# chechaohp/gan-ode

Hardware: AMD Instinct MI355X
Metric: generated videos/sec (16-frame clips) (higher is better)
Workload: dtype f32

## Files before the change

gan-ode_amd/_lib.py:

```python
from __future__ import annotations

import ctypes as C
import os

_HERE = os.path.dirname(os.path.abspath(__file__))
LIB_PATH = os.path.join(_HERE, "lib", "libgode.so")

i32, i64, f32, ptr = C.c_int32, C.c_int64, C.c_float, C.c_void_p
cint, u32, u64 = C.c_int, C.c_uint32, C.c_uint64

ACT_NONE, ACT_RELU, ACT_LRELU, ACT_TANH_OUT = 0, 1, 2, 3
ACT_TANH, ACT_SIGMOID = 4, 5
ACT_LRELU01 = 6
EPI_RAW, EPI_TANH = 0, 1
FPROP, DGRAD = 0, 1
PACK_BORDER = 0x100
OP_IGEMM, OP_WGRAD, OP_BN_FINALIZE, OP_BN_BWD, OP_ODE_FWD, OP_ODE_BWD, OP_BCE, OP_ADAM, OP_PACK = range(1, 10)
OP_ODERNN_FWD, OP_ODERNN_BWD, OP_BN_APPLY, OP_COL2IM = 10, 11, 12, 13
OP_SDE_FWD, OP_SDE_BWD = 14, 15
OP_CDE_FWD, OP_CDE_BWD = 16, 17
OP_WGAN = 18
OP_GRU_FWD, OP_GRU_BWD = 19, 20
OP_DNOISE = 21
OP_CATEG, OP_CE = 22, 23
OP_CHSTATS, OP_CBN_EMBED, OP_CBN_EMBED_BWD, OP_CBN_APPLY, OP_CBN_BWD, OP_GRES_OUT, OP_GRES_OUT_BWD, OP_SN_FWD, OP_SN_BWD = range(24, 33)
OP_FC_ACT, OP_FC_ACT_BWD, OP_BCE_PROB = 33, 34, 35
OP_BCE_T = 36
OP_RESIZE_U8, OP_CLIP_GATHER = 37, 38
RESIZE_MAX_TAPS = 32
REC_ADAM_NOISE = -1
ODE_NPARAM = 2672
ODERNN_NPARAM = 2176
SDE_NPARAM = 3216
CDE_NPARAM = 7536
CDE_MAX_N = 4096
GRU_NPARAM = 1632
# ... 315 lines not shown
    "gode_bn_bwd_work_size": ([i64, i32], i64),
    "gode_ode_bwd_work_size": ([i32], i64),
    "gode_odernn_bwd_work_size": ([i32], i64),
    "gode_odernn_sync_size": ([i32], i64),
    "gode_sde_bwd_work_size": ([i32], i64),
    "gode_cde_sync_size": ([i32], i64),
    "gode_cde_state_size": ([i32, i32], i64),
    "gode_cde_bwd_work_size": ([i32], i64),
    "gode_gru_bwd_work_size": ([i32], i64),
    "gode_ode_fwd_multi": ([ptr, i32, ptr], cint),
    "gode_ode_bwd_multi": ([ptr, i32, ptr], cint),
    "gode_odernn_fwd_multi": ([ptr, i32, ptr], cint),
    "gode_odernn_bwd_multi": ([ptr, i32, ptr], cint),
    "gode_odernn_fwd_route": ([ptr, i32, ptr], cint),
    "gode_odernn_bwd_route": ([ptr, i32, ptr], cint),
    "gode_gru_fwd_multi": ([ptr, i32, ptr], cint),
    "gode_gru_bwd_multi": ([ptr, i32, ptr], cint),
    "gode_chstats_rows": ([i64], cint),
    "gode_cbn_bwd_work_size": ([i32, i32, i32, i32], i64),
    "gode_gres_out_bwd_work_size": ([i32, i32, i32, i32, i32, i32], i64),
    "gode_fc_act_bwd_work_size": ([i64, i32], i64),
    "gode_dropout_mask": ([ptr, i64, u64, u32, f32, ptr], cint),
    "gode_scale": ([ptr, ptr, i64, f32, cint, ptr], cint),
    "gode_adam_multi": ([ptr, i32, i64, f32, f32, f32, f32, f32, f32, i32, ptr], cint),
    "gode_adam_multi_dev": ([ptr, i32, i64, f32, f32, f32, f32, f32, ptr, ptr], cint),
    "gode_adam_noise_multi": ([ptr, i32, i64, f32, f32, f32, f32, f32, f32, i32, u64, u32, u32, f32, ptr], cint),
    "gode_adam_noise_multi_dev": ([ptr, i32, i64, f32, f32, f32, f32, f32, ptr, u64, u32, f32, ptr], cint),
    "gode_param_noise": ([ptr, i64, u64, u32, u32, i64, f32, i32, ptr], cint),
    "gode_dnoise_normals": ([ptr, i64, u64, u32, u32, u32, i64, i32, ptr], cint),
    "gode_ode_step_chunks": ([ptr, i64], i64),
    "gode_ode_step": ([ptr, i32, i64, i32, f32, f32, f32, f32, f32, ptr, ptr], cint),
    "gode_axpy_multi": ([ptr, i32, i64, f32, ptr, ptr, f32, ptr, ptr, ptr], cint),
    "gode_run": ([ptr, ptr, i32, ptr], cint),
    "gode_version": (None, cint),
    "gode_sizeof": ([cint], cint),
}

EXPORTS = [st.FN for st in _OPS] + list(_PROTOS)

_lib = None


def lib():
    global _lib
    if _lib is not None:
        return _lib
    if not os.path.exists(LIB_PATH):
        raise RuntimeError(f"{LIB_PATH} is missing: build it with `python __graft_entry__.py` "
                           "(hipcc --offload-arch=gfx950); there is no CPU or PyTorch fallback")
    L = C.CDLL(LIB_PATH)
    for name in EXPORTS:
        if not hasattr(L, name):
            raise RuntimeError(f"libgode.so does not export {name}")
        fn = getattr(L, name)
        fn.argtypes, fn.restype = _PROTOS.get(name, ([ptr, ptr], cint))
    for kind, st in _STRUCTS.items():
        if L.gode_sizeof(kind) != C.sizeof(st):
            raise RuntimeError(f"ABI mismatch for op kind {kind}: C {L.gode_sizeof(kind)} != ctypes {C.sizeof(st)}")
    _lib = L
    return L


def check(rc, what="gode call"):
    if rc != 0:
        raise RuntimeError(f"{what} failed with code {rc}" + (" (hipError)" if rc > 0 else " (argument/shape error)"))


TRACE = None


def _traced(op, stream, launch):
    import torch
    e0, e1 = torch.cuda.Event(enable_timing=True), torch.cuda.Event(enable_timing=True)
    e0.record()
    launch()
    e1.record()
    TRACE.append((op, e0, e1))


def call(tag, launch):
    if TRACE is not None:
        return _traced(tag, None, launch)
    launch()


class Program:

    def __init__(self, ops):
        self.ops = list(ops)
        n = len(self.ops)
        self.kinds = (i32 * n)(*[op.KIND for op in self.ops])
        self.ptrs = (ptr * n)(*[C.addressof(op) for op in self.ops])
        self.n = n

    def run(self, stream):
        if TRACE is not None:
            for op in self.ops:
                run_one(op, stream)
            return
        check(lib().gode_run(self.kinds, self.ptrs, self.n, stream), "gode_run")


def run_one(op, stream):
    if op.KIND == OP_PACK:
        launch = lambda: check(lib().gode_pack_weights(C.byref(op.g), op.dir, op.w, op.wpack, op.co_perm, op.co_canon,
                                                       stream), "gode_pack_weights")
        return _traced(op, stream, launch) if TRACE is not None else launch()
    if TRACE is not None:
        return _traced(op, stream, lambda: _run_one(op, stream))
    _run_one(op, stream)


def _run_one(op, stream):
    check(getattr(lib(), op.FN)(C.byref(op), stream), op.FN)
```

gan-ode_amd/csrc/api.hip:

```cpp
#include "common.h"

extern "C" int gode_version(void) { return GODE_VERSION; }

extern "C" int gode_sizeof(int kind) {
  switch (kind) {
    case 0: return (int)sizeof(gode_conv_geom);
    case -1: return (int)sizeof(gode_adam_noise_tensor);
    case GODE_OP_PACK: return (int)sizeof(gode_pack_op);
#define GODE_SIZEOF_ROW_(name, value, op_t, fn) case GODE_OP_##name: return (int)sizeof(op_t);
    GODE_OPS(GODE_SIZEOF_ROW_)
#undef GODE_SIZEOF_ROW_
  }
  return GODE_E_KIND;
}

extern "C" int gode_pack_batch_(const gode_pack_op* const* ops, int n, void* stream);

extern "C" int gode_run(const int32_t* kinds, const void* const* ops, int32_t n, void* stream) {
  if (n < 0 || (n > 0 && (!kinds || !ops))) return GODE_E_ARG;
  for (int i = 0; i < n; ++i) {
    int rc;
    switch (kinds[i]) {
#define GODE_RUN_ROW_(name, value, op_t, fn) case GODE_OP_##name: rc = fn((const op_t*)ops[i], stream); break;
      GODE_OPS(GODE_RUN_ROW_)
#undef GODE_RUN_ROW_
      case GODE_OP_PACK: {
        int j = i;
        while (j + 1 < n && kinds[j + 1] == GODE_OP_PACK) ++j;
        rc = gode_pack_batch_((const gode_pack_op* const*)(ops + i), j - i + 1, stream);
        if (rc == 0) i = j;
        break;
      }
      default: return GODE_E_KIND;
    }
    if (rc != 0) return rc > 0 ? rc : rc * 1000 - i;
  }
  return 0;
}
```

gan-ode_amd/engine.py:

```python
from __future__ import annotations

import ctypes as C
import os
from dataclasses import dataclass
from typing import List, Optional, Sequence

import numpy as np
import torch

from . import _lib as L

BORDER_TAKE_DEAD_TAPS = 0.06
BORDER_TAKE_TILES_PER_SLOT = 2.0


def border_value(g) -> int:
    lib = L.lib()
    if lib.gode_igemm_dead_taps(C.byref(L.IgemmOp(g=g, dir=L.DGRAD, tile=0))) < BORDER_TAKE_DEAD_TAPS:
        return 1
    info = (C.c_int32 * 4)()
    L.check(lib.gode_igemm_launch_info(C.byref(L.IgemmOp(g=g, dir=L.DGRAD, tile=0, border=2)), info))
    return 2 if info[0] and info[2] >= BORDER_TAKE_TILES_PER_SLOT * info[3] else 1


def make_geom(N, Ci, Co, xi, yo, k, s, p) -> L.ConvGeom:
    return L.ConvGeom(N, Ci, Co, xi[0], xi[1], xi[2], yo[0], yo[1], yo[2], k[0], k[1], k[2], s[0], s[1], s[2],
                      p[0], p[1], p[2])


def conv_out(i, k, s, p):
    return (i + 2 * p - k) // s + 1


def dptr(t: Optional[torch.Tensor]):
    return None if t is None else t.data_ptr()


def stream_ptr():
    return torch.cuda.current_stream().cuda_stream


@dataclass
class LayerSpec:
    geom: L.ConvGeom
    fwd_dir: int
    act: int
    has_bn: bool
    epilogue: int = L.EPI_RAW
    co_perm: Optional[torch.Tensor] = None
    noise: bool = False

    def out_dims(self):
        g = self.geom
        if self.fwd_dir == L.FPROP:
            return (g.N, g.Do, g.Ho, g.Wo, g.Co)
        return (g.N, g.Di, g.Hi, g.Wi, g.Ci)

    def in_dims(self):
        g = self.geom
        if self.fwd_dir == L.FPROP:
            return (g.N, g.Di, g.Hi, g.Wi, g.Ci)
        return (g.N, g.Do, g.Ho, g.Wo, g.Co)


@dataclass
class LayerParams:
    weight: torch.Tensor
    gamma: Optional[torch.Tensor] = None
    beta: Optional[torch.Tensor] = None
    running_mean: Optional[torch.Tensor] = None
    running_var: Optional[torch.Tensor] = None
    num_batches_tracked: Optional[torch.Tensor] = None
# ... 84 lines not shown
        self._param_ptrs = None

    def _shared_pack(self, l, direction, n):
        key = ("buf", l, direction)
        buf = self.pack_cache.get(key)
        if buf is None or buf.numel() != n or buf.device != torch.device(self.device):
            buf = self.pack_cache[key] = torch.empty(n, dtype=torch.float32, device=self.device)
            self.pack_cache.pop(("ver", l, direction), None)
        return buf

    def _attach_work(self, igemm_ops):
        lib = L.lib()
        need = max([lib.gode_igemm_work_size(C.byref(op)) for op in igemm_ops] + [0])
        if need > 0:
            if self._ig_work is None or self._ig_work.numel() < need:
                self._ig_work = torch.empty(need, dtype=torch.float32, device=self.device)
                for prog_ops in getattr(self, "_all_igemm", []):
                    for op in prog_ops:
                        op.work = self._ig_work.data_ptr()
            for op in igemm_ops:
                op.work = self._ig_work.data_ptr()
        self.__dict__.setdefault("_all_igemm", []).append(list(igemm_ops))

    def _run_stale_packs(self, packs, st):
        stale = []
        for l, d, op in packs:
            w = self.params[l].weight
            ver = (w._version, getattr(w, "_gode_ver", 0), w.data_ptr())
            if self.pack_cache.get(("ver", l, d)) != ver:
                self.pack_cache[("ver", l, d)] = ver
                stale.append(op)
        if stale:
            L.Program(stale).run(st)

    @staticmethod
    def _ncols(s: LayerSpec):
        g = s.geom
        if s.fwd_dir == L.FPROP:
            return g.Co
        fullk = (g.Do == 1 and g.Ho == 1 and g.Wo == 1 and g.pd == 0 and g.ph == 0 and g.pw == 0 and
                 g.Di == g.kd and g.Hi == g.kh and g.Wi == g.kw and g.kd * g.kh * g.kw > 1)
        return g.kd * g.kh * g.kw * g.Ci if fullk else g.Ci

    def _materialize(self, l):
        if l + 1 >= len(self.specs):
            return False
        if self.specs[l + 1].noise:
            return True
        prod, cons = self.specs[l], self.specs[l + 1]
        C_out = prod.out_dims()[4]
        g = cons.geom
        taps = g.kd * g.kh * g.kw
        macs = g.N * g.Do * g.Ho * g.Wo * g.Co * g.Ci * taps
        heavy = C_out % 32 == 0 and macs >= (1 << 30) and (prod.has_bn or prod.act != L.ACT_NONE)
        if self._G2 and prod.has_bn:
            if self.split and not heavy and l + 1 == self.nl - 1 and cons.epilogue == L.EPI_TANH and not cons.has_bn:
                self._last_parts = True
                return False
            return True
        return heavy

    def _head_as_gemm(self, l):
        s = self.specs[l]
        g = s.geom
        taps = g.kh * g.kw
        pixels = g.N * g.Ho * g.Wo
# ... 223 lines not shown
                    continue
                ops.append(L.BnApplyOp(y=dptr(self.y[l]), out=dptr(self.a[l]), scale=dptr(self.scale[l]),
                                       shift=dptr(self.shift[l]), M=M, C=d[4], act=s.act, M0=M0))
        patch["packs"] = packs
        self._attach_work([op for op in ops if isinstance(op, L.IgemmOp)])
        return L.Program(ops), patch

    def _noise_op(self, noise, l, scale, shift, M0):
        d = self.specs[l].out_dims()
        op = L.DnoiseOp(x=dptr(self.y[l]), out=dptr(self.a[l]), scale=scale, shift=shift, M=d[0] * d[1] * d[2] * d[3],
                        C=d[4], act=self.specs[l].act, M0=M0, layer=l + 1)
        noise.append((op, d[1] * d[2] * d[3] * d[4], 0, None))
        return op

    @staticmethod
    def _patch_noise(patch, noise, inputs):
        seed = int(noise["seed"]) & 0xFFFFFFFFFFFFFFFF
        seed = seed - (1 << 64) if seed >= 1 << 63 else seed
        dev = noise.get("call_dev")
        base = 0 if dev else int(noise["call"])
        for op, per, add, k in patch["noise"]:
            op.seed, op.stream, op.sigma = seed, int(noise["stream"]), float(noise["sigma"])
            c = (base + add) & 0xFFFFFFFF
            op.call_dev, op.call = dev, c - (1 << 32) if c >= 1 << 31 else c
            op.e_off = int(noise.get("sample_offset", 0)) * per
            if k is not None:
                x, xs = inputs[k]
                op.x = x.data_ptr()
                for i in range(5):
                    op.xs[i] = int(xs[i])

    def forward(self, training: bool, x: Optional[torch.Tensor] = None, x_strides=None, pre_ops_program=None,
                x2: Optional[torch.Tensor] = None, x2_strides=None, noise=None):
        self._refresh()
        if training not in self._fwd:
            self._fwd[training] = self._build_fwd(training)
        prog, patch = self._fwd[training]
        if self.noisy:
            if noise is None:
                raise RuntimeError("this plan applies instance noise: forward() needs its noise arguments")
            self._patch_noise(patch, noise, [(x, x_strides), (x2, x2_strides)])
        out = torch.empty(self.out_dims, dtype=torch.float32, device=self.device)
        patch["last"].out = out.data_ptr()
        if "last2" in patch:
            patch["last2"][0].out = out.data_ptr() + patch["last2"][1]
        if self.x_in is None and self.x0n is None:
            first = patch["first"]
            first.src = x.data_ptr()
            for i in range(5):
                first.gs[i] = int(x_strides[i])
        if self.x_in is None:
            self._x_user, self._x_strides = x.detach(), tuple(int(v) for v in x_strides)
            if self.groups == 2:
                if self.x0n is None:
                    second = patch["first2"]
                    second.src = x2.data_ptr()
                    for i in range(5):
                        second.gs[i] = int(x2_strides[i])
                self._x2_user, self._x2_strides = x2.detach(), tuple(int(v) for v in x2_strides)
        st = stream_ptr()
        self._run_stale_packs(patch["packs"], st)
        if pre_ops_program is not None:
            pre_ops_program.run(st)
        prog.run(st)
        self.out = out.detach()
        self.generation += 1
        self._fwd_training = training
        return out

    def n_grad_floats(self):
        n = 0
        for p in self.params:
            n += p.weight.numel()
            if p.gamma is not None:
                n += p.gamma.numel() + p.beta.numel()
        return n

    def _build_bwd(self, need_input_grad: bool, need_param_grad: bool = True, training: bool = True):
        lib = L.lib()
        f32 = dict(dtype=torch.float32, device=self.device)
        if self.g is None:
            self.g = [torch.empty(s.out_dims(), **f32) for s in self.specs]
            self.g_in = None
        ops, patch = [], {"dw": [], "dgamma": [], "dbeta": []}
        bpacks = []
        wg_work = 0
        bn_work = 0
        last = self.specs[-1]
        readers = patch["gout_readers"] = []
        if last.epilogue == L.EPI_TANH:
            M = self._count(self.nl - 1)
            op = L.BnBwdOp(g=dptr(self.g[-1]), y=None, M=M, C=last.out_dims()[4], act=L.ACT_TANH_OUT)
            patch["tanh"] = op
            readers.append((op, "gin"))
            ops.append(op)
        for l in range(self.nl - 1, -1, -1):
            s, p = self.specs[l], self.params[l]
# ... 229 lines not shown
```

gan-ode_amd/modules.py:

```python
from __future__ import annotations

import ctypes as C
import math
from typing import Optional

import numpy as np
import torch
import torch.nn as nn

from . import _lib as L
from .engine import ConvStack, LayerParams, LayerSpec, conv_out, dptr, make_geom, stream_ptr

Z_COLS = 96
Z_CATEG0 = 66
MAX_CATEG = Z_COLS - Z_CATEG0
ODE_METHODS = L.ODE_METHODS


def ode_method_code(name):
    return L.ode_method_code(name)


def _require_gpu(t: torch.Tensor, what: str):
    if not t.is_cuda:
        raise RuntimeError(f"{what}: this implementation runs only on an MI355X through libgode.so; move the module "
                           "to the GPU with .cuda() (there is no CPU or PyTorch fallback)")


class _Pool:

    MAX_PLANS = 6

    def __init__(self):
        self.plans = {}
        self.pack_cache = {}

    def get(self, key, factory):
        lst = self.plans.setdefault(key, [])
        for p in lst:
            if not p.busy:
                return p
        if len(lst) >= self.MAX_PLANS:
            p = lst.pop(0)
            p.busy = False
            lst.append(p)
            return p
        p = factory()
        lst.append(p)
        return p
# ... 165 lines not shown
    multi, multi_always = ("ode", L.OdeFwdOp, L.OdeBwdOp), False

    def __init__(self, gen: "VideoGenerator", n_traj: int, T: int, select: bool, zbuf=None, x=None):
        dev = gen.main[0].weight.device
        self.gen, self.n, self.T, self.select, self.device = gen, n_traj, T, select, dev
        self.rows = n_traj if select else n_traj * T
        f32 = dict(dtype=torch.float32, device=dev)
        self.ncat = int(getattr(gen, "dim_z_category", 0)) if x is None else 0
        self.labels = None
        self.x, self.content, self.sel, self.cls = x, None, None, None
        self._ring = []
        if x is None:
            xs = self._x_shape(n_traj, T)
            sx, sc, ss, sk = _input_slices(int(np.prod(xs)), n_traj)
            nin = sk.stop if self.ncat else sk.start
            self._in = torch.zeros(nin, **f32)
            self.x, self.content = self._in[sx].view(xs), self._in[sc].view(n_traj, 50)
            self.sel = self._in[ss].view(torch.int32) if select else None
            self.cls = self._in[sk].view(torch.int32) if self.ncat else None
            self._ring = [dict(buf=torch.zeros(nin).pin_memory(), ev=None) for _ in range(4)]
        self._ring_i = 0
        self.stack = None
        if x is not None:
            self._zbuf, self._zcols = torch.empty(n_traj * T, self.zcols, **f32), self.zcols
        elif zbuf is not None:
            self._zbuf, self._zcols = zbuf, Z_COLS
        else:
            self.stack = ConvStack(gen._decoder_specs(self.rows), gen._decoder_params(), dev, owns_input=True,
                                   pack_cache=gen._pool.pack_cache, two_lane_backward=True)
            self._zbuf, self._zcols = self.stack.x_in, Z_COLS
        self._alloc()
        self._ode_ptrs = None
        self.busy = False

    @staticmethod
    def _x_shape(n_traj, T):
        return (n_traj, 16)

    def _alloc(self):
        f32 = dict(dtype=torch.float32, device=self.device)
        self.traj = torch.empty(self.n, self.T, 16, **f32)
        tt = torch.linspace(0, 1, self.T).float()
        self.dt = (tt[1:] - tt[:-1]).to(self.device) if self.T > 1 else torch.zeros(1, **f32)
        self.ode_work = torch.empty(L.lib().gode_ode_bwd_work_size(self.n), **f32)

    def _params(self):
        g = self.gen
        lin = g.linear
        if isinstance(lin, nn.Identity):
            pre = (None, None, None, None)
        else:
            pre = (lin[0].weight, lin[0].bias, lin[2].weight, lin[2].bias)
        return pre + tuple(_ode_fn_tensors(g.ode_fn))

    @classmethod
    def multi_ok(cls, gen, adjoint):
        if cls.multi is None:
            return False
        return cls.multi_always or (gen.ode_method == "dopri5" and not (adjoint and gen.adjoint_substeps != 0))

    def check_solve(self):
        """Host-side look at a finished solve (the CDE plan's: it raises when the kernel stopped early)."""

    def latent_rows(self):
        if self.rows_in_traj:
            return self.traj.view(self.n * self.T, 16)
# ... 52 lines not shown
                                          rows_per=1 if self.select else self.T, C=self.ncat, zcols=zcols, col0=Z_CATEG0)
            self.fwd_prog = L.Program([self.fwd_op] + ([self.categ_op] if self.ncat else []))
        self.fwd_op.substeps = self.bwd_op.substeps = self.gen.ode_substeps
        if self.gen.ode_method == "dopri5":
            self.bwd_op.substeps = self.gen.adjoint_substeps

    def stage_inputs(self, x_host, content_host, sel_host, cls_host=None):
        self._programs()
        if self.ncat:
            if cls_host is None:
                raise RuntimeError("a categorical generator plan needs the classes of its trajectories")
            if getattr(self.gen, "_feed", None) is not None and self.gen._feed.recording:
                raise NotImplementedError("categorical latents are not captured in a graph (GanTrainer(graph=True))")
            if not self.select:
                self.labels = torch.empty(self.n, dtype=torch.int64, device=self.device)
            self.categ_op.labels_out = dptr(self.labels) if not self.select else None
        feed = getattr(self.gen, "_feed", None)
        if feed is not None and feed.recording:
            nfl = self._in.numel()
            pin, dev = feed.noise_region(self.gen, self.select, self.n, self.T, nfl)
            _pack_inputs(pin, x_host, content_host, sel_host, cls_host)
            self._in.copy_(dev)
        else:
            slot = self._ring[self._ring_i]
            self._ring_i = (self._ring_i + 1) % len(self._ring)
            if slot["ev"] is not None:
                slot["ev"].synchronize()
            _pack_inputs(slot["buf"], x_host, content_host, sel_host, cls_host)
            self._in.copy_(slot["buf"], non_blocking=True)
            if slot["ev"] is None:
                slot["ev"] = torch.cuda.Event()
            slot["ev"].record()

    def forward(self, x_host, content_host, sel_host, training, keep, cls_host=None):
        if x_host is None:
            torch.cuda.current_stream().wait_event(self._latent_ev)
            out = self.stack.forward(training)
        else:
            self.stage_inputs(x_host, content_host, sel_host, cls_host)
            out = self.stack.forward(training, pre_ops_program=self.fwd_prog)
        self.busy = keep
        return out

    def _decoder_pass_done(self):
        cb = getattr(self.gen, "_on_decoder_grads", None)
        if cb is not None:
            self.gen._decoder_passes_left -= 1
            if self.gen._decoder_passes_left == 0:
                cb()

    def backward(self, gout, arena=None):
        if arena is not None:
            into = _grads_into(arena, self.gen._decoder_params())
            _, _, gz = self.stack.backward(gout, need_input_grad=True, into=into)
            self._decoder_pass_done()
            self.latent_backward(gz.data_ptr(), arena, gz)
            self.busy = False
            return None, None
        flat, views, gz = self.stack.backward(gout, need_input_grad=True)
        motion = self.latent_backward(gz.data_ptr(), None, gz)
        self.busy = False
        return views, motion

    def latent_backward(self, gz_ptr, arena, keep):
        op = self.bwd_op
        op.gz = gz_ptr
        ps = self._params()
        absent = _PRENET_NPARAM if ps[0] is None else 0
        cut = absent if self.grads_from_first_present else 0
        if arena is not None:
            tgt = [arena.target(q) for q in ps if q is not None]
            base, acc = tgt[0]
            op.grads = base.data_ptr() - 4 * (absent - cut)
            op.accumulate = 1 if acc else 0
            batch = getattr(self.gen, "_adjoint_batch", None)
# ... 69 lines not shown
        return (None,) * (n_other + ctx.n_params)
    views, motion = plan.backward(gout, None)
    grads = _flat_grads(views)
    assert len(grads) == ctx.n_dec and len(motion) == ctx.n_params - ctx.n_dec
    return (None,) * n_other + (*grads, *motion)


class _GenJointFn(torch.autograd.Function):

    @staticmethod
    def forward(ctx, plan, host, training, keep, n_dec, *params):
        out = plan.forward(host, training, keep)
        ctx.plan, ctx.n_dec, ctx.n_params = plan, n_dec, len(params)
        ctx.lease = _Lease(plan)
        ctx.out_shape = tuple(out.shape)
        return out.narrow(0, 0, plan.rows_v), out.narrow(0, plan.rows_v, plan.rows_i)

    @staticmethod
    def backward(ctx, gv, gi):
        plan = ctx.plan
        ctx.lease.check(type(plan.gen).__name__ + " (joint pass)")
        g = torch.empty(ctx.out_shape, dtype=torch.float32, device=plan.device)
        for part, gg in ((g.narrow(0, 0, plan.rows_v), gv), (g.narrow(0, plan.rows_v, plan.rows_i), gi)):
            if gg is None:
                part.zero_()
            else:
                part.copy_(gg)
        return _gen_backward(ctx, plan, g, 5)


class _GenFn(torch.autograd.Function):

    @staticmethod
    def forward(ctx, plan, x_host, content_host, sel_host, cls_host, training, keep, n_dec, *params):
        out = plan.forward(x_host, content_host, sel_host, training, keep, cls_host)
        ctx.plan, ctx.n_dec, ctx.n_params = plan, n_dec, len(params)
        ctx.lease = _Lease(plan)
        return out

    @staticmethod
    def backward(ctx, gout):
        plan = ctx.plan
        ctx.lease.check(type(plan.gen).__name__)
        return _gen_backward(ctx, plan, gout, 8)


class _LatentFn(torch.autograd.Function):

    @staticmethod
    def forward(ctx, gen, x_host, n, T, *params):
        lp = gen._plan_cls(gen, n, T, False, x=x_host.to(gen.main[0].weight.device))
        lp._programs()
        lp.fwd_prog.run(stream_ptr())
        lp.check_solve()
        ctx.lp = lp
        return lp.latent_rows()

    @staticmethod
    def backward(ctx, gout):
        lp = ctx.lp
        g = gout.contiguous()
        lp.bwd_op.zcols = 16
        return (None, None, None, None, *lp.latent_backward(g.data_ptr(), None, g))


class VideoGenerator(nn.Module):

    mnist = False
    _plan_cls = None
    _categorical_ok = True
    _one_layer_ok = True
    ode_method = "rk4"
    ode_rtol, ode_atol, adjoint_substeps = 1e-7, 1e-9, 0

    def __init__(self, n_channels, dim_z_content, dim_z_category, dim_z_motion, video_length, ode_fn=ODEFunc,
                 dim_hidden=None, linear=True, ngf=64):
        super().__init__()
        if not self._categorical_ok and dim_z_category != 0:
            raise NotImplementedError(f"categorical latents (dim_z_category={dim_z_category}) are implemented for the "
                                      f"Neural-ODE generators only, not for {type(self).__name__}")
        if not (0 <= int(dim_z_category) <= MAX_CATEG) or int(dim_z_category) != dim_z_category:
            raise NotImplementedError(f"dim_z_category={dim_z_category}: the categorical one-hot lives in the {MAX_CATEG} pad "
                                      f"columns of the {Z_COLS}-column latent row (0 <= dim_z_category <= {MAX_CATEG})")
        if dim_z_motion != 16 or dim_z_content != 50:
            raise NotImplementedError("libgode's fused ODE kernels are specialised for dim_z_motion=16, "
                                      "dim_z_content=50 (mnist_moco_ode.py:78, ucf_moco_ode.py:80)")
        self.n_channels, self.dim_z_content, self.dim_z_category = n_channels, dim_z_content, dim_z_category
        self.dim_z_motion, self.video_length, self.ngf = dim_z_motion, video_length, ngf
        self.ode_substeps = 1
        self.ode_step_size = None
        dim_z = dim_z_motion + dim_z_category + dim_z_content
        self.recurrent = nn.GRUCell(dim_z_motion, dim_z_motion)
        self.main = self._make_main(dim_z, ngf, n_channels, mnist=False)
        self._init_ode_parts(ode_fn, dim_hidden, linear, dim_z, ngf)
        self._pool = _Pool()

    def _init_ode_parts(self, ode_fn, dim_hidden, linear, dim_z, ngf):
        if dim_hidden is None and not (isinstance(ode_fn, type) and _is_one_layer(ode_fn)):
            raise TypeError("ODEFunc.__init__() missing 1 required positional argument: 'dim_hidden' "
                            "(pass dim_hidden=16; ucf_moco_ode.py:80 omits it and fails the same way)")
        self.ode_fn = self._make_ode_fn(ode_fn, dim_hidden)
        self.linear = self._make_prenet(linear)
# ... 67 lines not shown
            specs.append(LayerSpec(make_geom(rows, nc, ngf, (1, 64, 64), (1, 32, 32), (1, 4, 4), (1, 2, 2), (0, 1, 1)),
                                   L.DGRAD, L.ACT_NONE, False, epilogue=L.EPI_TANH))
        return specs

    def _decoder_params(self):
        m = self.main
        out = []
        for i in range(4):
            conv, bn = m[3 * i], m[3 * i + 1]
            out.append(LayerParams(conv.weight, bn.weight, bn.bias, bn.running_mean, bn.running_var,
                                   bn.num_batches_tracked))
        out.append(LayerParams(m[12].weight))
        return out

    def _decoder_list(self):
        return _flat_params(self._decoder_params())

    def _param_list(self):
        ode = []
        if not isinstance(self.linear, nn.Identity):
            ode += [self.linear[0].weight, self.linear[0].bias, self.linear[2].weight, self.linear[2].bias]
        ode += _ode_fn_tensors(self.ode_fn)
        return self._decoder_list(), ode

    def _apply(self, fn, *a, **k):
        r = super()._apply(fn, *a, **k)
        if hasattr(self, "_pool"):
            self._pool.clear()
            self.__dict__.pop("_labels", None)
            self.__dict__.pop("_latent_plans", None)
            self.__dict__.pop("_prefetched", None)
        return r

    def invalidate_packs(self):
        for k in [k for k in self._pool.pack_cache if k[0] == "ver"]:
            del self._pool.pack_cache[k]

    def _zero_labels(self, n, device):
        key = (n, device)
        t = self.__dict__.setdefault("_labels", {}).get(key)
        if t is None:
            t = self._labels[key] = torch.zeros(n, dtype=torch.float64, device=device)
        return t

    _gode_direct_grads = True

    def _arena_tail(self):
        return self._param_list()[1]

    def _draw(self, num_samples, video_len):
        content = np.random.normal(0, 1, (num_samples, self.dim_z_content)).astype(np.float32)
        x = torch.randn(num_samples, self.dim_z_motion)
        return torch.from_numpy(content), x

    def _run(self, n_traj, T, select, x, content, sel, cls=None, plan=None):
        _require_gpu(self.main[0].weight, type(self).__name__)
        if plan is None:
            plan = self._pool.get((n_traj, T, select), lambda: self._plan_cls(self, n_traj, T, select))
        dec, ode = self._param_list()
        keep = torch.is_grad_enabled() and any(p.requires_grad for p in dec + ode)
        return _GenFn.apply(plan, x, content, sel, cls, self.training, keep, len(dec), *dec, *ode)

    def prefetch_latents(self, calls):
        _require_gpu(self.main[0].weight, type(self).__name__)
        if self.__dict__.get("_prefetched"):
            raise RuntimeError("prefetch_latents: the previous prefetch has not been consumed "
                               f"({len(self._prefetched)} calls left)")
        for kind, n in calls:
            if kind not in ("videos", "images", "pair_vi", "pair_iv"):
                raise ValueError(f"prefetch_latents: unknown call kind {kind!r}")
        main = torch.cuda.current_stream()
        lat = self.__dict__.get("_latent_stream")
        if lat is None or lat.device != main.device:
            lat = self._latent_stream = torch.cuda.Stream(device=main.device)
        plans, queue = [], []
        T = self.video_length
        per_shape = {}
        for kind, n in calls:
            per_shape[(kind, n)] = per_shape.get((kind, n), 0) + 1
        if max(per_shape.values(), default=0) > _Pool.MAX_PLANS:
            raise RuntimeError(f"prefetch_latents: more than {_Pool.MAX_PLANS} calls of one shape ahead (each holds its own "
                               "plan and buffers); announce fewer calls at a time")
        for kind, n in calls:
            if kind.startswith("pair"):
                plan = self._joint_plan(n[0], n[1], T, kind == "pair_iv")
                if plan is None:
                    raise RuntimeError(f"prefetch_latents: {kind}{n} cannot be decoded jointly; announce the two calls")
                plan.busy = True
                plans.append(plan)
                queue.append((kind, n, T, plan))
                continue
            select = kind == "images"
            plan = self._pool.get((n, T, select), lambda: self._plan_cls(self, n, T, select))
            plan.busy = True
# ... 624 lines not shown
        self.last_counts = None

    def _x_shape(self, n_traj, T):
        return (n_traj, T)

    def _params(self):
        g = self.gen
        f, fn = g.f, g.ode_fn
        return (f[0].weight, f[0].bias, f[2].weight, f[2].bias, fn.linear1.weight, fn.linear1.bias,
                fn.linear2.weight, fn.linear2.bias)

    def _programs(self):
        ps = self._params()
        key = tuple(dptr(p) for p in ps) + (self.gen.cde_rtol, self.gen.cde_atol)
        if key != self._ode_ptrs:
            self._ode_ptrs = key
            common = dict(p=L.CdeParams(*key[:8]), x=dptr(self.x), tslope=dptr(self.tslope), sel_t=dptr(self.sel),
                          states=dptr(self.states), sched=dptr(self.sched), counts=dptr(self.counts), N=self.n,
                          T=self.T, S_cap=self.S_cap, zcols=self._zcols)
            self.fwd_op = L.CdeFwdOp(content=dptr(self.content), z=dptr(self._zbuf), sync=dptr(self.sync),
                                     rtol=float(self.gen.cde_rtol), atol=float(self.gen.cde_atol), **common)
            self.bwd_op = L.CdeBwdOp(gz=None, work=dptr(self.cde_work), grads=None, accumulate=0, **common)
            self.fwd_prog = L.Program([self.fwd_op])

    def check_solve(self):
        c = self.counts.cpu().tolist()
        self.last_counts = c
        if c[0] < 0:
            raise RuntimeError(f"{type(self.gen).__name__}: the dopri5 CDE solve stopped after {-c[0] - 1} accepted steps "
                               f"({c[1]} trials): more than cde_max_steps = {self.S_cap} accepted steps, or the step "
                               "size underflowed; raise cde_max_steps or loosen cde_rtol / cde_atol")
        return c

    def forward(self, x_host, content_host, sel_host, training, keep, cls_host=None):
        if x_host is None:
            return super().forward(None, content_host, sel_host, training, keep)
        self.stage_inputs(x_host, content_host, sel_host, cls_host)
        self.fwd_prog.run(stream_ptr())
        self.check_solve()
        out = self.stack.forward(training)
        self.busy = keep
        return out


class VideoGeneratorCDE(VideoGeneratorMNIST):

    _categorical_ok = False

    _plan_cls = _CdeGenPlan
    _gode_graph_capture = False
    cde_rtol, cde_atol = 1e-4, 1e-6
    cde_max_steps = 512

    def __init__(self, n_channels, dim_z_content, dim_z_category, dim_z_motion, video_length, ode_fn=CDEFunc,
                 cde_input_dim=2, dim_hidden=None, linear=True, ngf=64):
        self._cde_args = (cde_input_dim, dim_hidden)
        super().__init__(n_channels, dim_z_content, dim_z_category, dim_z_motion, video_length, ode_fn=ode_fn,
                         dim_hidden=None, linear=linear, ngf=ngf)

    def _init_ode_parts(self, ode_fn, dim_hidden, linear, dim_z, ngf):
        cde_input_dim, dim_hidden = self._cde_args
        del self._cde_args
        if cde_input_dim != 2:
            raise NotImplementedError(f"cde_input_dim={cde_input_dim}: the path of models/mocogan_cde.py is [time, noise] "
                                      "(2 channels), the only one libgode's fused CDE kernels integrate")
        if dim_hidden not in (None, 16):
            raise NotImplementedError(f"dim_hidden={dim_hidden}: libgode's fused CDE kernels are specialised for the "
# ... 290 lines not shown
```

gan-ode_amd/train.py:

```python
from __future__ import annotations

import contextlib
from typing import List, Optional, Sequence

import torch
import torch.distributed as dist

from . import _lib as L
from .engine import stream_ptr
from .modules import PatchImageDiscriminator, VideoDiscriminator, VideoGenerator, VideoGeneratorMNISTODE


def host_cpu_quota():
    import os
    n = len(os.sched_getaffinity(0)) if hasattr(os, "sched_getaffinity") else (os.cpu_count() or 1)
    try:
        quota, period = open("/sys/fs/cgroup/cpu.max").read().split()[:2]
        if quota != "max":
            n = min(n, max(1, int(int(quota) / int(period))))
    except Exception:
        pass
    return n


# ... 771 lines not shown
            if self.world > 1:
                self._all_reduce(a.flat, False)
            opt.step(gscale=gscale, feed=feed)
            return
        if self.world > 1:
            b = self.buckets[id(model)]
            b.gather()
            b.all_reduce(self.group)
            opt.step(grads=b.views(), gscale=gscale)
        else:
            opt.step(gscale=gscale)

    def _d_loss(self, pr, pf):
        if self.loss == "wasserstein":
            return wasserstein_discriminator_loss(pr, pf)
        return bce_with_logits_pair(pr, 1.0, pf, 0.0)

    def _d_loss_joint(self, joint):
        if self.loss == "wasserstein":
            return wasserstein_discriminator_loss_halves(joint)
        return bce_with_logits_halves(joint, 1.0, 0.0)

    @staticmethod
    def _mean(losses):
        if len(losses) == 1:
            return losses[0]
        return torch.stack(losses).mean()

    def _noise_shard(self, model, k, B, nsh, call0):
        if getattr(model, "use_noise", False):
            model._noise_call = call0
            model._noise_sample_offset = (self.rank * nsh + k) * B

    def d_image_step(self, real_img, _join=True, _defer=False, _pair_videos=0):
        shards = _shards(real_img)
        side = self._side
        main = torch.cuda.current_stream() if side is not None else None
        if side is not None and not self._side_pending:
            side.wait_stream(main)
            self._side_pending = True
        on_side = (lambda: torch.cuda.stream(side)) if side is not None else contextlib.nullcontext
        with on_side():
            self._begin(self.dis_img, self.img_opt)
        losses = []
        call0 = getattr(self.dis_img, "_noise_call", 0)
        for k, x in enumerate(shards):
            B = x.shape[0]
            self._noise_shard(self.dis_img, k, B, len(shards), call0)
            if not self.pair_d:
                with on_side():
                    pr, _ = self.dis_img(x)
            with torch.no_grad():
                if _pair_videos:
                    self._paired_fake_vid, (fake, _) = self.gen.sample_pair(_pair_videos, B, images_first=True)
                else:
                    fake, _ = self.gen.sample_images(B)
            if side is not None:
                ev = torch.cuda.Event()
                ev.record(main)
                side.wait_event(ev)
                fake.record_stream(side)
            with on_side():
                if self.pair_d:
                    loss = self._d_loss_joint(self.dis_img.forward_pair_joint(x, fake))
                else:
                    pf, _ = self.dis_img(fake)
                    loss = self._d_loss(pr, pf)
                loss.backward(gradient=unit_grad(loss.device))
            losses.append(loss.detach())
        with on_side():
            self._opt_step(self.dis_img, self.img_opt, len(shards))
            if not _defer:
                self._flush(self.dis_img)
            out = self._mean(losses)
        if _join:
            self._join_side()
        return out

    def _join_side(self):
        if self._side is not None and self._side_pending:
            torch.cuda.current_stream().wait_stream(self._side)
            self._side_pending = False

    def _labels_for(self, real_labels, B, what):
        if not self.ncat:
            if real_labels is not None:
                raise ValueError(f"{what}: real_labels given, but the networks are unconditional (dim_z_category=0)")
            return None
        if real_labels is None:
            raise ValueError(f"{what}: categorical training (dim_z_category={self.ncat}) needs real_labels, the int64 "
                             "class of every real video")
        if not (torch.is_tensor(real_labels) and real_labels.dtype == torch.int64 and real_labels.dim() == 1
                and real_labels.shape[0] == B and real_labels.is_cuda):
            raise ValueError(f"{what}: real_labels must be an int64 device tensor [{B}]")
        return real_labels

    def d_video_step(self, real_vid, _defer=False, real_labels=None):
        shards = _shards(real_vid)
        if self.ncat and len(shards) > 1:
            raise NotImplementedError("categorical training does not take virtual-replica shards")
        labels = self._labels_for(real_labels, shards[0].shape[0], "d_video_step")
        losses = []
        begun = False
        call0 = getattr(self.dis_vid, "_noise_call", 0)
        for k, x in enumerate(shards):
            B = x.shape[0]
            self._noise_shard(self.dis_vid, k, B, len(shards), call0)
            real = x.transpose(1, 2)
            if not self.pair_d and not begun:
                self._begin(self.dis_vid, self.vid_opt)
                begun = True
            if not self.pair_d:
                pr = self.dis_vid.forward_head(real) if self.ncat else self.dis_vid(real)[0]
            with torch.no_grad():
                fake, self._paired_fake_vid = self._paired_fake_vid, None
                if fake is not None:
                    fake = fake[0]
                    assert fake.shape[0] == B
                else:
                    fake, _ = self.gen.sample_videos(B)
            if not begun:
                self._begin(self.dis_vid, self.vid_opt)
                begun = True
            if self.ncat:
                if self.pair_d:
                    loss = bce_ce_head_halves(self.dis_vid.forward_pair_joint(real, fake), 1.0, 0.0, labels)
                else:
                    loss = bce_ce_heads(pr, 1.0, labels, self.dis_vid.forward_head(fake), 0.0)
            elif self.pair_d:
                loss = self._d_loss_joint(self.dis_vid.forward_pair_joint(real, fake))
            else:
                pf, _ = self.dis_vid(fake)
                loss = self._d_loss(pr, pf)
            loss.backward(gradient=unit_grad(loss.device))
            losses.append(loss.detach())
        self._opt_step(self.dis_vid, self.vid_opt, len(shards))
        if not _defer:
            self._flush(self.dis_vid)
        return self._mean(losses)

    def _can_pair(self, n_videos, n_images, images_first):
        return self.joint_g and hasattr(self.gen, "can_pair") and next(self.gen.parameters()).is_cuda and \
            self.gen.can_pair(n_videos, n_images, images_first)

    def g_step(self, B, shards=1):
        if self.ncat and shards > 1:
            raise NotImplementedError("categorical training does not take virtual-replica shards")
# ... 172 lines not shown
```

include/gode.h:

```cpp
#ifndef GODE_H
#define GODE_H
#include <stdint.h>
#ifdef __cplusplus
extern "C" {
#endif

#define GODE_VERSION 105

enum { GODE_OK = 0, GODE_E_ARG = -1, GODE_E_SHAPE = -2, GODE_E_KIND = -3 };
enum { GODE_ACT_NONE = 0, GODE_ACT_RELU = 1, GODE_ACT_LRELU = 2,
       GODE_ACT_TANH_OUT = 3 ,
       GODE_ACT_TANH = 4, GODE_ACT_SIGMOID = 5 ,
       GODE_ACT_LRELU01 = 6  };
enum { GODE_EPI_RAW = 0, GODE_EPI_TANH = 1 };
enum { GODE_FPROP = 0, GODE_DGRAD = 1 };
enum { GODE_PACK_BORDER = 0x100 };

typedef struct gode_conv_geom {
  int32_t N, Ci, Co;
  int32_t Di, Hi, Wi;
  int32_t Do, Ho, Wo;
  int32_t kd, kh, kw;
  int32_t sd, sh, sw;
  int32_t pd, ph, pw;
// ... 386 lines not shown
  X(SDE_FWD,       14, gode_sde_fwd_op,       gode_sde_fwd)       \
  X(SDE_BWD,       15, gode_sde_bwd_op,       gode_sde_bwd)       \
  X(CDE_FWD,       16, gode_cde_fwd_op,       gode_cde_fwd)       \
  X(CDE_BWD,       17, gode_cde_bwd_op,       gode_cde_bwd)       \
  X(WGAN,          18, gode_wgan_op,          gode_wgan_logits)   \
  X(GRU_FWD,       19, gode_gru_fwd_op,       gode_gru_fwd)       \
  X(GRU_BWD,       20, gode_gru_bwd_op,       gode_gru_bwd)       \
  X(DNOISE,        21, gode_dnoise_op,        gode_dnoise)        \
  X(CATEG,         22, gode_categ_op,         gode_categ_onehot)  \
  X(CE,            23, gode_ce_op,            gode_ce_logits)     \
  X(CHSTATS,       24, gode_chstats_op,       gode_chstats)       \
  X(CBN_EMBED,     25, gode_cbn_embed_op,     gode_cbn_embed)     \
  X(CBN_EMBED_BWD, 26, gode_cbn_embed_bwd_op, gode_cbn_embed_bwd) \
  X(CBN_APPLY,     27, gode_cbn_apply_op,     gode_cbn_apply)     \
  X(CBN_BWD,       28, gode_cbn_bwd_op,       gode_cbn_bwd)       \
  X(GRES_OUT,      29, gode_gres_out_op,      gode_gres_out)      \
  X(GRES_OUT_BWD,  30, gode_gres_out_bwd_op,  gode_gres_out_bwd)  \
  X(SN_FWD,        31, gode_sn_op,            gode_sn_fwd)        \
  X(SN_BWD,        32, gode_sn_bwd_op,        gode_sn_bwd)        \
  X(FC_ACT,        33, gode_fc_act_op,        gode_fc_act)        \
  X(FC_ACT_BWD,    34, gode_fc_act_bwd_op,    gode_fc_act_bwd)    \
  X(BCE_PROB,      35, gode_bce_prob_op,      gode_bce_prob)      \
  X(BCE_T,         36, gode_bce_t_op,         gode_bce_logits_t)  \
  X(RESIZE_U8,     37, gode_resize_u8_op,     gode_resize_u8)     \
  X(CLIP_GATHER,   38, gode_clip_gather_op,   gode_clip_gather)
#define GODE_ENUM_ROW_(name, value, op_t, fn) GODE_OP_##name = value,
enum { GODE_OPS(GODE_ENUM_ROW_) GODE_OP_PACK = 9 };
#undef GODE_ENUM_ROW_
typedef struct gode_pack_op {
  gode_conv_geom g; int32_t dir , co_canon; const float* w; float* wpack; const int32_t* co_perm;
} gode_pack_op;
int gode_run(const int32_t* kinds, const void* const* ops, int32_t n, void* stream);

int gode_version(void);
int gode_sizeof(int kind);

#ifdef __cplusplus
}
#endif
#endif
```

Baseline: 38780.

## Overlap next sample's ODE front ops with previous generator tail on a side stream

Adds a two-lane execution path for no-grad generator sampling. The front of the program (input staging, ODE forward and the first conv) runs on a dedicated side HIP stream. The rest runs on the main stream, and events release the side lane once the last reader of the front's outputs has run. Consecutive sampling calls can then overlap the next call's front with the previous call's tail, hiding serial latency. The cost is added event and stream bookkeeping, pointer-overlap dependency analysis, and a risk of races if the write sets are incomplete.

```diff
diff --git a/gan-ode_amd/_lib.py b/gan-ode_amd/_lib.py
--- a/gan-ode_amd/_lib.py
+++ b/gan-ode_amd/_lib.py
@@ -2,6 +2,7 @@
 
 import ctypes as C
 import os
+import sys
 
 _HERE = os.path.dirname(os.path.abspath(__file__))
 LIB_PATH = os.path.join(_HERE, "lib", "libgode.so")
@@ -383,6 +384,10 @@
     "gode_ode_step": ([ptr, i32, i64, i32, f32, f32, f32, f32, f32, ptr, ptr], cint),
     "gode_axpy_multi": ([ptr, i32, i64, f32, ptr, ptr, f32, ptr, ptr, ptr], cint),
     "gode_run": ([ptr, ptr, i32, ptr], cint),
+    "gode_lanes_create": ([ptr], cint),
+    "gode_lanes_destroy": ([ptr], cint),
+    "gode_lanes_stream": ([ptr], ptr),
+    "gode_run_lanes": ([ptr, ptr, ptr, i32, i32, i32, i32, ptr], cint),
     "gode_version": (None, cint),
     "gode_sizeof": ([cint], cint),
 }
@@ -429,7 +434,12 @@
     TRACE.append((op, e0, e1))
 
 
+LAUNCHES = 0
+
+
 def call(tag, launch):
+    global LAUNCHES
+    LAUNCHES += 1
     if TRACE is not None:
         return _traced(tag, None, launch)
     launch()
@@ -445,6 +455,8 @@
         self.n = n
 
     def run(self, stream):
+        global LAUNCHES
+        LAUNCHES += 1
         if TRACE is not None:
             for op in self.ops:
                 run_one(op, stream)
@@ -452,7 +464,45 @@
         check(lib().gode_run(self.kinds, self.ptrs, self.n, stream), "gode_run")
 
 
+LANES_ORDERED, LANES_OVERLAP = 0, 1
+
+
+class Lanes:
+
+    _free = {}
+
+    def __init__(self, device_index):
+        self.device_index = device_index
+        pool = Lanes._free.setdefault(device_index, [])
+        if pool:
+            self.handle = pool.pop()
+        else:
+            self.handle = ptr()
+            check(lib().gode_lanes_create(C.byref(self.handle)), "gode_lanes_create")
+        self.stream_ptr = lib().gode_lanes_stream(self.handle)
+
+    def __del__(self):
+        h, self.handle = getattr(self, "handle", None), None
+        if h and not sys.is_finalizing():
+            Lanes._free.setdefault(self.device_index, []).append(h)
+
+
+class LanesProgram(Program):
+
+    def __init__(self, ops, n_front, release_after):
+        super().__init__(ops)
+        self.n_front, self.release_after = int(n_front), int(release_after)
+
+    def run_lanes(self, lanes, mode, stream):
+        global LAUNCHES
+        LAUNCHES += 1
+        check(lib().gode_run_lanes(lanes.handle, self.kinds, self.ptrs, self.n, self.n_front, self.release_after, mode,
+                                   stream), "gode_run_lanes")
+
+
 def run_one(op, stream):
+    global LAUNCHES
+    LAUNCHES += 1
     if op.KIND == OP_PACK:
         launch = lambda: check(lib().gode_pack_weights(C.byref(op.g), op.dir, op.w, op.wpack, op.co_perm, op.co_canon,
                                                        stream), "gode_pack_weights")
diff --git a/gan-ode_amd/csrc/api.hip b/gan-ode_amd/csrc/api.hip
--- a/gan-ode_amd/csrc/api.hip
+++ b/gan-ode_amd/csrc/api.hip
@@ -16,9 +16,8 @@
 
 extern "C" int gode_pack_batch_(const gode_pack_op* const* ops, int n, void* stream);
 
-extern "C" int gode_run(const int32_t* kinds, const void* const* ops, int32_t n, void* stream) {
-  if (n < 0 || (n > 0 && (!kinds || !ops))) return GODE_E_ARG;
-  for (int i = 0; i < n; ++i) {
+static int run_range(const int32_t* kinds, const void* const* ops, int lo, int hi, void* stream) {
+  for (int i = lo; i < hi; ++i) {
     int rc;
     switch (kinds[i]) {
 #define GODE_RUN_ROW_(name, value, op_t, fn) case GODE_OP_##name: rc = fn((const op_t*)ops[i], stream); break;
@@ -26,7 +25,7 @@
 #undef GODE_RUN_ROW_
       case GODE_OP_PACK: {
         int j = i;
-        while (j + 1 < n && kinds[j + 1] == GODE_OP_PACK) ++j;
+        while (j + 1 < hi && kinds[j + 1] == GODE_OP_PACK) ++j;
         rc = gode_pack_batch_((const gode_pack_op* const*)(ops + i), j - i + 1, stream);
         if (rc == 0) i = j;
         break;
@@ -37,3 +36,90 @@
   }
   return 0;
 }
+
+extern "C" int gode_run(const int32_t* kinds, const void* const* ops, int32_t n, void* stream) {
+  if (n < 0 || (n > 0 && (!kinds || !ops))) return GODE_E_ARG;
+  return run_range(kinds, ops, 0, n, stream);
+}
+
+struct gode_lanes {
+  hipStream_t side;
+  hipEvent_t ev_entry, ev_front, ev_release;
+  bool released;
+};
+
+#define GODE_HIP_TRY(expr)                          \
+  do {                                              \
+    hipError_t e__ = (expr);                        \
+    if (e__ != hipSuccess) return (int)e__;         \
+  } while (0)
+
+extern "C" int gode_lanes_destroy(gode_lanes* l) {
+  if (!l) return GODE_E_ARG;
+  int rc = 0;
+  if (l->side) {
+    hipError_t e = hipStreamSynchronize(l->side);
+    if (e != hipSuccess) rc = (int)e;
+  }
+  hipEvent_t evs[3] = {l->ev_entry, l->ev_front, l->ev_release};
+  for (hipEvent_t ev : evs)
+    if (ev) { hipError_t e = hipEventDestroy(ev); if (e != hipSuccess && rc == 0) rc = (int)e; }
+  if (l->side) { hipError_t e = hipStreamDestroy(l->side); if (e != hipSuccess && rc == 0) rc = (int)e; }
+  delete l;
+  return rc;
+}
+
+extern "C" int gode_lanes_create(gode_lanes** out) {
+  if (!out) return GODE_E_ARG;
+  *out = nullptr;
+  gode_lanes* l = new gode_lanes();
+  hipError_t e = hipStreamCreateWithFlags(&l->side, hipStreamNonBlocking);
+  if (e == hipSuccess) e = hipEventCreateWithFlags(&l->ev_entry, hipEventDisableTiming);
+  if (e == hipSuccess) e = hipEventCreateWithFlags(&l->ev_front, hipEventDisableTiming);
+  if (e == hipSuccess) e = hipEventCreateWithFlags(&l->ev_release, hipEventDisableTiming);
+  if (e == hipSuccess) e = hipEventRecord(l->ev_front, l->side);
+  if (e != hipSuccess) {
+    gode_lanes_destroy(l);
+    return (int)e;
+  }
+  *out = l;
+  return 0;
+}
+
+extern "C" void* gode_lanes_stream(gode_lanes* l) { return l ? (void*)l->side : nullptr; }
+
+extern "C" int gode_run_lanes(gode_lanes* l, const int32_t* kinds, const void* const* ops, int32_t n, int32_t n_front,
+                              int32_t release_after, int32_t mode, void* stream) {
+  if (!l || n < 0 || (n > 0 && (!kinds || !ops)) || n_front < 0 || n_front > n || release_after < n_front ||
+      release_after >= n || (mode != GODE_LANES_ORDERED && mode != GODE_LANES_OVERLAP))
+    return GODE_E_ARG;
+  hipStream_t main = (hipStream_t)stream;
+  hipStreamCaptureStatus cap = hipStreamCaptureStatusNone;
+  if (hipStreamIsCapturing(main, &cap) != hipSuccess) {
+    (void)hipGetLastError();
+    cap = hipStreamCaptureStatusActive;
+  }
+  if (cap != hipStreamCaptureStatusNone) {
+    l->released = false;
+    return run_range(kinds, ops, 0, n, stream);
+  }
+  const bool overlap = mode == GODE_LANES_OVERLAP && l->released;
+  l->released = false;
+  if (overlap) {
+    GODE_HIP_TRY(hipStreamWaitEvent(l->side, l->ev_release, 0));
+  } else {
+    GODE_HIP_TRY(hipEventRecord(l->ev_entry, main));
+    GODE_HIP_TRY(hipStreamWaitEvent(l->side, l->ev_entry, 0));
+  }
+  int rc = run_range(kinds, ops, 0, n_front, (void*)l->side);
+  if (rc != 0) return rc;
+  GODE_HIP_TRY(hipEventRecord(l->ev_front, l->side));
+  GODE_HIP_TRY(hipStreamWaitEvent(main, l->ev_front, 0));
+  rc = run_range(kinds, ops, n_front, release_after + 1, stream);
+  if (rc != 0) return rc;
+  GODE_HIP_TRY(hipEventRecord(l->ev_release, main));
+  l->released = true;
+  rc = run_range(kinds, ops, release_after + 1, n, stream);
+  if (rc != 0) l->released = false;
+  return rc;
+}
diff --git a/gan-ode_amd/engine.py b/gan-ode_amd/engine.py
--- a/gan-ode_amd/engine.py
+++ b/gan-ode_amd/engine.py
@@ -38,6 +38,68 @@
 
 def stream_ptr():
     return torch.cuda.current_stream().cuda_stream
+
+
+_FRONT_WRITES = {L.OdeFwdOp: ("z", "traj"), L.IgemmOp: ("out", "stats", "work")}
+
+
+def op_pointers(op):
+    out = []
+    for name, tp in op._fields_:
+        v = getattr(op, name)
+        if tp is L.ptr:
+            if v:
+                out.append(v)
+        elif isinstance(v, C.Structure):
+            out += op_pointers(v)
+    return out
+
+
+def front_writes(front_ops, uses_work=lambda op: True):
+    written = set()
+    for op in front_ops:
+        fields = _FRONT_WRITES.get(type(op))
+        if fields is None:
+            raise ValueError(f"{type(op).__name__} has no write set: it cannot run on the side lane")
+        for f in fields:
+            v = getattr(op, f)
+            if v and (f != "work" or uses_work(op)):
+                written.add(v)
+    return written
+
+
+def release_after(ops, n_front, written=None, extents=None):
+    if not 0 < n_front < len(ops):
+        raise ValueError(f"a two-lane program needs ops on both lanes (n_front={n_front} of {len(ops)})")
+    if written is None:
+        written = front_writes(ops[:n_front])
+    spans = [(a, a + max(1, (extents or {}).get(a, 1))) for a in written]
+    last = n_front
+    for i in range(n_front, len(ops)):
+        if any(lo <= p < hi for p in op_pointers(ops[i]) for lo, hi in spans):
+            last = i
+    return last
+
+
+LANE_SINGLE, LANE_ORDERED, LANE_OVERLAP = "single", "ordered", "overlap"
+
+
+def ring_back(i, n, back):
+    return (i - back) % n
+
+
+def lane_gate(prev_lanes, prev_copy_pending, before_prev_copy_pending):
+    return bool(prev_copy_pending) if prev_lanes else bool(before_prev_copy_pending)
+
+
+def lane_mode(*, enabled, trace, recording, categorical, grad, keep, fixed_grid_ode, splittable, prev_lanes, launches_between,
+              repacked, versions_same, same_stream, gpu_behind=True):
+    if (not enabled or trace or recording or categorical or grad or keep or not fixed_grid_ode or not splittable
+            or not gpu_behind):
+        return LANE_SINGLE
+    if prev_lanes and launches_between == 0 and not repacked and versions_same and same_stream:
+        return LANE_OVERLAP
+    return LANE_ORDERED
 
 
 @dataclass
@@ -188,6 +250,20 @@
                 stale.append(op)
         if stale:
             L.Program(stale).run(st)
+        return bool(stale)
+
+    def front_split(self, prog, pre_ops):
+        first = prog.ops[0] if prog.ops else None
+        if (self.split or self.groups != 1 or self.noisy or self.x_in is None or len(prog.ops) < 2
+                or not isinstance(first, L.IgemmOp) or first.out != dptr(self.y[0])):
+            return None
+        lib = L.lib()
+        ops = list(pre_ops) + list(prog.ops)
+        n_front = len(pre_ops) + 1
+        written = front_writes(ops[:n_front], uses_work=lambda op: lib.gode_igemm_work_size(C.byref(op)) > 0)
+        extents = {t.data_ptr(): t.numel() * t.element_size()
+                   for t in (self.x_in, self.y[0], self.stats[0], self._ig_work) if t is not None}
+        return ops, n_front, release_after(ops, n_front, written, extents)
 
     @staticmethod
     def _ncols(s: LayerSpec):
@@ -477,6 +553,14 @@
 
     def forward(self, training: bool, x: Optional[torch.Tensor] = None, x_strides=None, pre_ops_program=None,
                 x2: Optional[torch.Tensor] = None, x2_strides=None, noise=None):
+        prog, out, _ = self.begin_forward(training, x, x_strides, x2, x2_strides, noise)
+        st = stream_ptr()
+        if pre_ops_program is not None:
+            pre_ops_program.run(st)
+        prog.run(st)
+        return self.end_forward(out, training)
+
+    def begin_forward(self, training: bool, x=None, x_strides=None, x2=None, x2_strides=None, noise=None):
         self._refresh()
         if training not in self._fwd:
             self._fwd[training] = self._build_fwd(training)
@@ -503,11 +587,9 @@
                     for i in range(5):
                         second.gs[i] = int(x2_strides[i])
                 self._x2_user, self._x2_strides = x2.detach(), tuple(int(v) for v in x2_strides)
-        st = stream_ptr()
-        self._run_stale_packs(patch["packs"], st)
-        if pre_ops_program is not None:
-            pre_ops_program.run(st)
-        prog.run(st)
+        return prog, out, self._run_stale_packs(patch["packs"], stream_ptr())
+
+    def end_forward(self, out, training):
         self.out = out.detach()
         self.generation += 1
         self._fwd_training = training
diff --git a/gan-ode_amd/modules.py b/gan-ode_amd/modules.py
--- a/gan-ode_amd/modules.py
+++ b/gan-ode_amd/modules.py
@@ -1,7 +1,9 @@
 from __future__ import annotations
 
+import contextlib
 import ctypes as C
 import math
+import os
 from typing import Optional
 
 import numpy as np
@@ -9,12 +11,14 @@
 import torch.nn as nn
 
 from . import _lib as L
-from .engine import ConvStack, LayerParams, LayerSpec, conv_out, dptr, make_geom, stream_ptr
+from .engine import (LANE_ORDERED, LANE_OVERLAP, LANE_SINGLE, ConvStack, LayerParams, LayerSpec, conv_out, dptr, lane_gate,
+                     lane_mode, make_geom, ring_back, stream_ptr)
 
 Z_COLS = 96
 Z_CATEG0 = 66
 MAX_CATEG = Z_COLS - Z_CATEG0
 ODE_METHODS = L.ODE_METHODS
+_SAMPLE_LANES_ENV = os.environ.get("GODE_SAMPLE_LANES", "1") != "0"
 
 
 def ode_method_code(name):
@@ -246,6 +250,12 @@
         self._alloc()
         self._ode_ptrs = None
         self.busy = False
+        self._lanes = self._side = self._lane_prog = self._lane_prev = None
+        self.lane_calls = {LANE_OVERLAP: 0, LANE_ORDERED: 0, LANE_SINGLE: 0}
+        self._lanes_ok = type(self) is _GenPlan and self.stack is not None and not self.ncat and _SAMPLE_LANES_ENV
+        self.lanes_made_late = False
+        if self._lanes_ok and gen.sample_lanes:
+            self._make_lanes()
 
     @staticmethod
     def _x_shape(n_traj, T):
@@ -364,15 +374,93 @@
                 slot["ev"] = torch.cuda.Event()
             slot["ev"].record()
 
-    def forward(self, x_host, content_host, sel_host, training, keep, cls_host=None):
+    def forward(self, x_host, content_host, sel_host, training, keep, cls_host=None, no_grad=False):
         if x_host is None:
             torch.cuda.current_stream().wait_event(self._latent_ev)
             out = self.stack.forward(training)
+            self._lane_prev = None
+        elif self._lanes_possible(keep, no_grad):
+            out = self._forward_lanes(x_host, content_host, sel_host, training)
         else:
             self.stage_inputs(x_host, content_host, sel_host, cls_host)
             out = self.stack.forward(training, pre_ops_program=self.fwd_prog)
+            self._lane_prev = None
+            self.lane_calls[LANE_SINGLE] += 1
         self.busy = keep
         return out
+
+    def _lanes_possible(self, keep, no_grad):
+        gen = self.gen
+        if (not no_grad or keep or not gen.sample_lanes or gen._one_stream or not self._lanes_ok or L.TRACE is not None
+                or gen.ode_method == "dopri5"):
+            return False
+        if gen.sample_lanes != "always" and not lane_gate(self._lane_prev is not None, self._copy_pending(1),
+                                                          self._copy_pending(2)):
+            return False
+        feed = getattr(gen, "_feed", None)
+        if (feed is not None and feed.recording) or torch.cuda.is_current_stream_capturing():
+            return False
+        if self._lanes is None:
+            self._make_lanes()
+            self.lanes_made_late = True
+        return True
+
+    def _copy_pending(self, back):
+        ev = self._ring[ring_back(self._ring_i, len(self._ring), back)]["ev"]
+        return ev is not None and not ev.query()
+
+    def _make_lanes(self):
+        with torch.cuda.device(self.device):
+            self._lanes = L.Lanes(torch.cuda.current_device())
+        self._side = torch.cuda.ExternalStream(self._lanes.stream_ptr, device=self.device)
+
+    def _front_versions(self):
+        ts = [t for t in self._params() if t is not None] + [self.stack.params[0].weight]
+        return tuple((t._version, getattr(t, "_gode_ver", 0), t.data_ptr()) for t in ts)
+
+    def _forward_lanes(self, x_host, content_host, sel_host, training):
+        self._programs()
+        prev, self._lane_prev = self._lane_prev, None
+        between = L.LAUNCHES - prev["mark"] if prev is not None else -1
+        prog, out, repacked = self.stack.begin_forward(training)
+        st = stream_ptr()
+        cache = self._lane_prog
+        if cache is None or cache[0] is not prog or cache[1] is not self.fwd_prog:
+            split = self.stack.front_split(prog, self.fwd_prog.ops)
+            cache = self._lane_prog = (prog, self.fwd_prog, None if split is None else L.LanesProgram(*split))
+            prev = None
+        lp = cache[2]
+        versions = self._front_versions()
+        mode = lane_mode(enabled=True, trace=False, recording=False, categorical=False, grad=False, keep=False,
+                         fixed_grid_ode=True, splittable=lp is not None, prev_lanes=prev is not None,
+                         launches_between=between, repacked=repacked,
+                         versions_same=prev is not None and prev["versions"] == versions,
+                         same_stream=prev is not None and prev["stream"] == st,
+                         gpu_behind=True)
+        self.lane_calls[mode] += 1
+        if mode == LANE_SINGLE:
+            self.stage_inputs(x_host, content_host, sel_host)
+            self.fwd_prog.run(st)
+            prog.run(st)
+        else:
+            self._stage_on_side(mode == LANE_ORDERED, x_host, content_host, sel_host)
+            lp.run_lanes(self._lanes, L.LANES_OVERLAP if mode == LANE_OVERLAP else L.LANES_ORDERED, st)
+            self._lane_prev = dict(mark=L.LAUNCHES, versions=versions, stream=st)
+        return self.stack.end_forward(out, training)
+
+    def _stage_on_side(self, ordered, x_host, content_host, sel_host):
+        slot = self._ring[self._ring_i]
+        self._ring_i = (self._ring_i + 1) % len(self._ring)
+        if slot["ev"] is not None:
+            slot["ev"].synchronize()
+        _pack_inputs(slot["buf"], x_host, content_host, sel_host)
+        if ordered:
+            self._side.wait_stream(torch.cuda.current_stream())
+        with torch.cuda.stream(self._side):
+            self._in.copy_(slot["buf"], non_blocking=True)
+            if slot["ev"] is None:
+                slot["ev"] = torch.cuda.Event()
+            slot["ev"].record()
 
     def _decoder_pass_done(self):
         cb = getattr(self.gen, "_on_decoder_grads", None)
@@ -508,8 +596,8 @@
 class _GenFn(torch.autograd.Function):
 
     @staticmethod
-    def forward(ctx, plan, x_host, content_host, sel_host, cls_host, training, keep, n_dec, *params):
-        out = plan.forward(x_host, content_host, sel_host, training, keep, cls_host)
+    def forward(ctx, plan, x_host, content_host, sel_host, cls_host, training, keep, no_grad, n_dec, *params):
+        out = plan.forward(x_host, content_host, sel_host, training, keep, cls_host, no_grad=no_grad)
         ctx.plan, ctx.n_dec, ctx.n_params = plan, n_dec, len(params)
         ctx.lease = _Lease(plan)
         return out
@@ -518,7 +606,7 @@
     def backward(ctx, gout):
         plan = ctx.plan
         ctx.lease.check(type(plan.gen).__name__)
-        return _gen_backward(ctx, plan, gout, 8)
+        return _gen_backward(ctx, plan, gout, 9)
 
 
 class _LatentFn(torch.autograd.Function):
@@ -544,6 +632,8 @@
 
     mnist = False
     _plan_cls = None
+    sample_lanes = True
+    _one_stream = 0
     _categorical_ok = True
     _one_layer_ok = True
     ode_method = "rk4"
@@ -677,9 +767,31 @@
             self.__dict__.pop("_prefetched", None)
         return r
 
+    def lane_stats(self):
+        out = {LANE_OVERLAP: 0, LANE_ORDERED: 0, LANE_SINGLE: 0, "lanes_objects": 0, "lanes_objects_made_late": 0}
+        for plans in self._pool.plans.values():
+            for p in plans:
+                for k, v in getattr(p, "lane_calls", {}).items():
+                    out[k] += v
+                out["lanes_objects"] += getattr(p, "_lanes", None) is not None
+                out["lanes_objects_made_late"] += bool(getattr(p, "lanes_made_late", False))
+        return out
+
+    @contextlib.contextmanager
+    def one_stream(self):
+        self._one_stream += 1
+        try:
+            yield
+        finally:
+            self._one_stream -= 1
+
     def invalidate_packs(self):
         for k in [k for k in self._pool.pack_cache if k[0] == "ver"]:
             del self._pool.pack_cache[k]
+        for plans in self._pool.plans.values():
+            for p in plans:
+                if getattr(p, "_lane_prev", None) is not None:
+                    p._lane_prev = None
 
     def _zero_labels(self, n, device):
         key = (n, device)
@@ -704,7 +816,8 @@
             plan = self._pool.get((n_traj, T, select), lambda: self._plan_cls(self, n_traj, T, select))
         dec, ode = self._param_list()
         keep = torch.is_grad_enabled() and any(p.requires_grad for p in dec + ode)
-        return _GenFn.apply(plan, x, content, sel, cls, self.training, keep, len(dec), *dec, *ode)
+        no_grad = not torch.is_grad_enabled()
+        return _GenFn.apply(plan, x, content, sel, cls, self.training, keep, no_grad, len(dec), *dec, *ode)
 
     def prefetch_latents(self, calls):
         _require_gpu(self.main[0].weight, type(self).__name__)
@@ -1395,7 +1508,7 @@
                                "size underflowed; raise cde_max_steps or loosen cde_rtol / cde_atol")
         return c
 
-    def forward(self, x_host, content_host, sel_host, training, keep, cls_host=None):
+    def forward(self, x_host, content_host, sel_host, training, keep, cls_host=None, no_grad=False):
         if x_host is None:
             return super().forward(None, content_host, sel_host, training, keep)
         self.stage_inputs(x_host, content_host, sel_host, cls_host)
diff --git a/gan-ode_amd/train.py b/gan-ode_amd/train.py
--- a/gan-ode_amd/train.py
+++ b/gan-ode_amd/train.py
@@ -827,6 +827,9 @@
             model._noise_call = call0
             model._noise_sample_offset = (self.rank * nsh + k) * B
 
+    def _gen_one_stream(self):
+        return getattr(self.gen, "one_stream", contextlib.nullcontext)()
+
     def d_image_step(self, real_img, _join=True, _defer=False, _pair_videos=0):
         shards = _shards(real_img)
         side = self._side
@@ -845,7 +848,7 @@
             if not self.pair_d:
                 with on_side():
                     pr, _ = self.dis_img(x)
-            with torch.no_grad():
+            with torch.no_grad(), self._gen_one_stream():
                 if _pair_videos:
                     self._paired_fake_vid, (fake, _) = self.gen.sample_pair(_pair_videos, B, images_first=True)
                 else:
@@ -907,7 +910,7 @@
                 begun = True
             if not self.pair_d:
                 pr = self.dis_vid.forward_head(real) if self.ncat else self.dis_vid(real)[0]
-            with torch.no_grad():
+            with torch.no_grad(), self._gen_one_stream():
                 fake, self._paired_fake_vid = self._paired_fake_vid, None
                 if fake is not None:
                     fake = fake[0]
diff --git a/include/gode.h b/include/gode.h
--- a/include/gode.h
+++ b/include/gode.h
@@ -442,6 +442,14 @@
 } gode_pack_op;
 int gode_run(const int32_t* kinds, const void* const* ops, int32_t n, void* stream);
 
+typedef struct gode_lanes gode_lanes;
+enum { GODE_LANES_ORDERED = 0, GODE_LANES_OVERLAP = 1 };
+int gode_lanes_create(gode_lanes** out);
+int gode_lanes_destroy(gode_lanes* lanes);
+void* gode_lanes_stream(gode_lanes* lanes);
+int gode_run_lanes(gode_lanes* lanes, const int32_t* kinds, const void* const* ops, int32_t n, int32_t n_front,
+                   int32_t release_after, int32_t mode, void* stream);
+
 int gode_version(void);
 int gode_sizeof(int kind);
 
```

Measured after the change: 39400 (median of 6 runs). +1.6%, better.
